# ViliamVadocz/takzero

Measured on AMD Instinct MI355X. Metric: mcts_simulations_per_s, higher is better.
Workload: dtype f16

## Files before the change

### bindings/takzero-hip-sys/src/lib.rs

```rust
#![allow(non_camel_case_types, clippy::too_many_arguments)]
use std::os::raw::{c_char, c_int, c_uint, c_void};

pub const TZ_MAX_N: c_int = 6;
pub const TZ_MAX_SQUARES: c_int = 36;
pub const TZ_MAX_ACTIONS: c_int = 512;
pub const TZ_MAX_ACTIONS_6: c_int = 1024;
pub const TZ_OK: c_int = 0;
pub const TZ_EINVAL: c_int = -1;
pub const TZ_EPARSE: c_int = -2;
pub const TZ_EDEVICE: c_int = -3;
pub const TZ_ENOMEM: c_int = -4;
pub const TZ_ECAPACITY: c_int = -5;
pub const TZ_ESTATE: c_int = -6;
pub const TZ_ENUMERIC: c_int = -7;
pub const TZ_EMPTY: c_int = 0;
pub const TZ_FLAT: c_int = 1;
pub const TZ_WALL: c_int = 2;
pub const TZ_CAP: c_int = 3;
pub const TZ_EVAL_VALUE: c_int = 0;
pub const TZ_EVAL_WIN: c_int = 1;
pub const TZ_EVAL_LOSS: c_int = 2;
pub const TZ_EVAL_DRAW: c_int = 3;
pub const TZ_TERMINAL_NONE: c_int = -1;
pub const TZ_TERMINAL_WIN: c_int = 0;
// ... 189 lines not shown
    pub fn tz_trainer_shape(t: *mut TzTrainer, board_n_out: *mut c_int, batch_out: *mut c_int, arch_out: *mut c_int) -> c_int;
    pub fn tz_trainer_load(t: *mut TzTrainer, path: *const c_char) -> c_int;
    pub fn tz_trainer_save(t: *mut TzTrainer, path: *const c_char) -> c_int;
    pub fn tz_trainer_load_weights_mem(t: *mut TzTrainer, data: *const c_void, bytes: usize) -> c_int;
    pub fn tz_trainer_get_extras(t: *mut TzTrainer, out: *mut c_void, cap: u64, bytes_out: *mut u64) -> c_int;
    pub fn tz_trainer_from_net(t: *mut TzTrainer, net: *mut TzNet) -> c_int;
    pub fn tz_trainer_to_net(t: *mut TzTrainer, net: *mut TzNet) -> c_int;
    pub fn tz_trainer_set_ensemble_targets(t: *mut TzTrainer, targets: *const f32) -> c_int;
    pub fn tz_trainer_ensemble_last(t: *mut TzTrainer, loss_out: *mut f32, values_out: *mut f32) -> c_int;
    pub fn tz_trainer_rnd_enable(t: *mut TzTrainer, on: c_int) -> c_int;
    pub fn tz_trainer_rnd_last(t: *mut TzTrainer, loss_out: *mut f32, raw_out: *mut f32) -> c_int;
    pub fn tz_trainer_rnd_activation(t: *mut TzTrainer, which: c_int, layer: c_int, out: *mut f32, out_cap: u64) -> c_int;
    pub fn tz_trainer_rnd_calibrate(t: *mut TzTrainer, early: *const TzState, n_early: c_int, late: *const TzState, n_late: c_int, apply: c_int, min_out: *mut f32, max_out: *mut f32) -> c_int;
    pub fn tz_trainer_rnd4_enable(t: *mut TzTrainer, on: c_int) -> c_int;
    pub fn tz_trainer_rnd4_last(t: *mut TzTrainer, loss_out: *mut f32, raw_out: *mut f32) -> c_int;
    pub fn tz_trainer_rnd4_activation(t: *mut TzTrainer, which: c_int, layer: c_int, out: *mut f32, out_cap: u64) -> c_int;
    pub fn tz_trainer_rnd4_calibrate(t: *mut TzTrainer, early: *const TzState, n_early: c_int, late: *const TzState, n_late: c_int, apply: c_int, min_out: *mut f32, max_out: *mut f32) -> c_int;
    pub fn tz_learn_create(trainer: *mut TzTrainer, half_komi: c_int, seed: u64, selfplay_forced_uses: c_int, reanalyze_forced_uses: c_int, out: *mut *mut TzLearn) -> c_int;
    pub fn tz_learn_destroy(l: *mut TzLearn) -> c_int;
    pub fn tz_learn_feed(l: *mut TzLearn, which: c_int, path: *const c_char, model_steps: c_int, added_out: *mut u64) -> c_int;
    pub fn tz_learn_add_lines(l: *mut TzLearn, which: c_int, text: *const c_char, len: u64, model_steps: c_int, added_out: *mut u64) -> c_int;
    pub fn tz_learn_buffer_len(l: *mut TzLearn, which: c_int, len_out: *mut u64) -> c_int;
    pub fn tz_learn_step(l: *mut TzLearn, using_reanalyze: c_int, train_ube: c_int, augment: c_int, losses_out: *mut f32) -> c_int;
    pub fn tz_learn_last_batch(l: *mut TzLearn, states_out: *mut TzState, policy_out: *mut f32, mask_out: *mut u8, value_out: *mut f32, ube_out: *mut f32) -> c_int;
    pub fn tz_learn_run(l: *mut TzLearn, directory: *const c_char, starting_steps: i64, steps: i64, min_selfplay: c_int, min_reanalyze: c_int, steps_before_reanalyze: i64, read_interval_s: f64, sleep_s: f64, wait_limit_s: f64, on_step: Option<unsafe extern "C" fn(*mut c_void, i64, *const f32, *const TzState, c_int) -> c_int>, user: *mut c_void, model_steps_out: *mut i64) -> c_int;
    pub fn tz_learn_set_save_points(l: *mut TzLearn, steps_per_save: c_int, steps_per_checkpoint: c_int, hash_net: *mut TzNet) -> c_int;
    pub fn tz_learn_set_rnd(l: *mut TzLearn, train_rnd: c_int, early: *const TzState, n_early: c_int, late: *const TzState, n_late: c_int, calibrate_every: c_int) -> c_int;
    pub fn tz_learn_rnd_reference(search: *mut TzSearch, seed: u64, n_early: c_int, early_ply: c_int, n_late: c_int, late_ply: c_int, early_out: *mut TzState, late_out: *mut TzState) -> c_int;
    pub fn tz_device_math(op: c_int, a: *const f32, b: *const f32, out: *mut f32, n: c_int) -> c_int;
    pub fn tz_debug_conv_bench(net: *mut TzNet, variant: c_int, positions: c_int, iters: c_int, ms_out: *mut f32) -> c_int;
    pub fn tz_debug_tower_bench(net: *mut TzNet, variant: c_int, positions: c_int, iters: c_int, ms_out: *mut f32) -> c_int;
    pub fn tz_debug_hash_bench(net: *mut TzNet, batch: c_int, states: *const TzState, iters: c_int, ms_out: *mut f32) -> c_int;
    pub fn tz_debug_rnd4_bench(net: *mut TzNet, batch: c_int, states: *const TzState, iters: c_int, ms_out: *mut f32) -> c_int;
    pub fn tz_debug_net_clock(net: *mut TzNet, mhz_out: *mut f64, tower_us_out: *mut f64) -> c_int;
    pub fn tz_debug_net_stamps(net: *mut TzNet, out: *mut u64, max_groups: c_int, groups_out: *mut c_int) -> c_int;
}
```

### include/takzero_hip.h

```cpp
#ifndef TAKZERO_HIP_H
#define TAKZERO_HIP_H

#include <stddef.h>
#include <stdint.h>

#ifdef __cplusplus
extern "C" {
#endif

#define TZ_MAX_N 6
#define TZ_MAX_SQUARES 36
#define TZ_MAX_ACTIONS 512
#define TZ_MAX_ACTIONS_6 1024

#define TZ_OK 0
#define TZ_EINVAL (-1)
#define TZ_EPARSE (-2)
#define TZ_EDEVICE (-3)
#define TZ_ENOMEM (-4)
#define TZ_ECAPACITY (-5)
#define TZ_ESTATE (-6)
#define TZ_ENUMERIC (-7)

#define TZ_EMPTY 0
// ... 220 lines not shown
int tz_trainer_rnd_activation(tz_trainer* t, int which, int layer, float* out, uint64_t out_cap);
int tz_trainer_rnd_calibrate(tz_trainer* t, const tz_state* early, int n_early, const tz_state* late, int n_late, int apply,
                             float* min_out, float* max_out);

int tz_trainer_rnd4_enable(tz_trainer* t, int on);
int tz_trainer_rnd4_last(tz_trainer* t, float* loss_out, float* raw_out );
int tz_trainer_rnd4_activation(tz_trainer* t, int which , int layer, float* out, uint64_t out_cap);
int tz_trainer_rnd4_calibrate(tz_trainer* t, const tz_state* early, int n_early, const tz_state* late, int n_late, int apply,
                              float* min_out, float* max_out);

typedef struct tz_learn tz_learn;
int tz_learn_create(tz_trainer* trainer, int half_komi, uint64_t seed, int selfplay_forced_uses, int reanalyze_forced_uses,
                    tz_learn** out);
int tz_learn_destroy(tz_learn* l);
int tz_learn_feed(tz_learn* l, int which, const char* path, int model_steps, uint64_t* added_out);
int tz_learn_add_lines(tz_learn* l, int which, const char* text, uint64_t len, int model_steps, uint64_t* added_out);
int tz_learn_buffer_len(tz_learn* l, int which, uint64_t* len_out);
int tz_learn_step(tz_learn* l, int using_reanalyze, int train_ube, int augment, float* losses_out);
int tz_learn_last_batch(tz_learn* l, tz_state* states_out, float* policy_out, uint8_t* mask_out, float* value_out, float* ube_out);
int tz_learn_run(tz_learn* l, const char* directory, int64_t starting_steps, int64_t steps, int min_selfplay, int min_reanalyze,
                 int64_t steps_before_reanalyze, double read_interval_s, double sleep_s, double wait_limit_s,
                 int (*on_step)(void*, int64_t, const float*, const tz_state*, int), void* user, int64_t* model_steps_out);
int tz_learn_set_save_points(tz_learn* l, int steps_per_save, int steps_per_checkpoint, tz_net* hash_net);
int tz_learn_set_rnd(tz_learn* l, int train_rnd, const tz_state* early, int n_early, const tz_state* late, int n_late,
                     int calibrate_every);
int tz_learn_rnd_reference(tz_search* search, uint64_t seed, int n_early, int early_ply, int n_late, int late_ply,
                           tz_state* early_out, tz_state* late_out);

int tz_device_math(int op, const float* a, const float* b, float* out, int n);
int tz_debug_conv_bench(tz_net* net, int variant, int positions, int iters, float* ms_out);
int tz_debug_tower_bench(tz_net* net, int variant, int positions, int iters, float* ms_out);
int tz_debug_hash_bench(tz_net* net, int batch, const tz_state* states, int iters, float* ms_out);
int tz_debug_rnd4_bench(tz_net* net, int batch, const tz_state* states, int iters, float* ms_out);
int tz_debug_net_clock(tz_net* net, double* mhz_out, double* tower_us_out);
int tz_debug_net_stamps(tz_net* net, unsigned long long* out, int max_groups, int* groups_out);

#ifdef __cplusplus
}
#endif
#endif
```

### takzero_amd/_lib.py

```python
import ctypes as C
import os

import numpy as np

HERE = os.path.dirname(os.path.abspath(__file__))
LIB_PATH = os.path.join(HERE, "libtakzero_hip.so")
MAX_SQ = 36

STATE_DTYPE = np.dtype([
    ("colors", np.uint64, (MAX_SQ,)), ("height", np.uint8, (MAX_SQ,)), ("top", np.uint8, (MAX_SQ,)),
    ("stones", np.uint8, (2,)), ("caps", np.uint8, (2,)), ("to_move", np.uint8), ("n", np.uint8),
    ("half_komi", np.int8), ("pad0", np.uint8), ("ply", np.uint16), ("reversible_plies", np.uint16),
], align=True)
ROOT_INFO_DTYPE = np.dtype([
    ("visit_count", np.uint32), ("n_children", np.uint32), ("eval_tag", np.uint8),
    ("is_terminal_env", np.uint8), ("ply", np.uint16), ("eval_bits", np.uint32),
    ("std_dev", np.float32), ("logit", np.float32), ("probability", np.float32)], align=True)
assert STATE_DTYPE.itemsize == 376 and ROOT_INFO_DTYPE.itemsize == 28

SYMBOLS = [
    "tz_last_error", "tz_version", "tz_device_count", "tz_state_from_tps", "tz_state_to_tps", "tz_move_to_ptn",
    "tz_move_from_ptn", "tz_policy_size", "tz_input_channels", "tz_net_create", "tz_net_load_weights",
    "tz_net_load_weights_mem", "tz_net_destroy", "tz_net_eval", "tz_net_encode", "tz_net_forward_raw", "tz_net_hash_indices", "tz_net_load_bitset", "tz_net_save_bitset",
    "tz_search_create", "tz_search_destroy", "tz_search_set_positions", "tz_search_get_positions",
    "tz_search_new_openings", "tz_search_simulate", "tz_search_apply_noise", "tz_search_root_info",
    "tz_search_root_children", "tz_search_node", "tz_search_select_best_actions", "tz_search_improved_policy", "tz_search_ube_target",
    "tz_search_step", "tz_search_restart_terminal", "tz_search_gumbel_sh", "tz_search_counters", "tz_search_sync", "tz_search_pool_usage",
    "tz_search_profile", "tz_device_math", "tz_debug_conv_bench", "tz_debug_tower_bench", "tz_debug_hash_bench", "tz_debug_rnd4_bench", "tz_net_ensemble_values", "tz_net_rnd_raw", "tz_net_load_prepare", "tz_net_load_commit", "tz_net_load_discard", "tz_debug_net_clock", "tz_debug_net_stamps", "tz_search_terminal_details", "tz_search_play_moves",
    "tz_trainer_set_ensemble_targets", "tz_trainer_ensemble_last", "tz_trainer_create", "tz_trainer_destroy", "tz_trainer_tensor_count", "tz_trainer_tensor_info",
    "tz_trainer_set_tensor", "tz_trainer_get_tensor", "tz_trainer_step", "tz_trainer_outputs", "tz_trainer_activation",
    "tz_format_targets", "tz_parse_targets", "tz_search_improved_policy_each", "tz_search_shape",
    "tz_selfplay_create", "tz_selfplay_destroy", "tz_selfplay_play_move", "tz_selfplay_counters", "tz_selfplay_take_text",
    "tz_selfplay_run", "tz_reanalyze_create", "tz_reanalyze_destroy", "tz_reanalyze_feed", "tz_reanalyze_iterate",
    "tz_reanalyze_take_text", "tz_reanalyze_run", "tz_compete", "tz_puzzle_benchmark", "tz_search_pool_overflows", "tz_trainer_shape",
    "tz_net_init_random", "tz_net_load_partial", "tz_net_save", "tz_net_clone", "tz_net_get_tensor", "tz_weights_convert", "tz_net_tensor_count", "tz_net_tensor_info",
    "tz_comm_unique_id", "tz_comm_rendezvous_id", "tz_comm_create_rccl", "tz_comm_create_fs", "tz_comm_destroy", "tz_comm_info",
    "tz_comm_all_gather", "tz_comm_take", "tz_comm_broadcast", "tz_comm_barrier", "tz_net_broadcast", "tz_selfplay_set_comm", "tz_selfplay_exchange",
    "tz_trainer_load", "tz_trainer_save", "tz_trainer_load_weights_mem", "tz_trainer_get_extras", "tz_trainer_from_net", "tz_trainer_to_net", "tz_learn_set_save_points",
    "tz_learn_create", "tz_learn_destroy", "tz_learn_feed", "tz_learn_add_lines", "tz_learn_buffer_len", "tz_learn_step", "tz_learn_run", "tz_learn_last_batch",
    "tz_search_simulate_batch", "tz_search_principal_variation", "tz_search_batch_profile",
    "tz_search_set_selection", "tz_search_get_selection",
    "tz_trainer_rnd_enable", "tz_trainer_rnd_last", "tz_trainer_rnd_activation", "tz_trainer_rnd_calibrate", "tz_learn_set_rnd",
    "tz_trainer_rnd4_enable", "tz_trainer_rnd4_last", "tz_trainer_rnd4_activation", "tz_trainer_rnd4_calibrate",
    "tz_learn_rnd_reference",
]

_lib = None


class TakzeroError(RuntimeError):
    def __init__(self, code, msg):
        super().__init__("libtakzero_hip error %d: %s" % (code, msg))
        self.code = code


def load():
    global _lib
    if _lib is not None:
        return _lib
    if not os.path.exists(LIB_PATH):
        try:
# ... 53 lines not shown
    lib.tz_search_set_positions.argtypes = [vp, ci, vp, vp]
    lib.tz_search_get_positions.argtypes = [vp, vp]
    lib.tz_search_new_openings.argtypes = [vp, vp]
    lib.tz_search_simulate.argtypes = [vp, vp, ci]
    lib.tz_search_simulate_batch.argtypes = [vp, vp, ci, ci]
    lib.tz_search_batch_profile.argtypes = [vp] + [C.POINTER(C.c_double)] * 3 + [C.POINTER(C.c_uint64)]
    lib.tz_search_set_selection.argtypes = [vp, ci]
    lib.tz_search_get_selection.argtypes = [vp, C.POINTER(ci)]
    lib.tz_search_principal_variation.argtypes = [vp, ci, vp, ci, C.POINTER(ci)]
    lib.tz_search_apply_noise.argtypes = [vp, vp, ci, cf]
    lib.tz_search_root_info.argtypes = [vp, vp]
    lib.tz_search_root_children.argtypes = [vp, ci] + [vp] * 7
    lib.tz_search_node.argtypes = [vp, ci, vp, ci, vp, ci] + [vp] * 7
    lib.tz_search_select_best_actions.argtypes = [vp, vp]
    lib.tz_search_improved_policy.argtypes = [vp, cf, ci, vp]
    lib.tz_search_improved_policy_each.argtypes = [vp, vp, ci, vp]
    lib.tz_search_ube_target.argtypes = [vp, cf, vp]
    lib.tz_search_step.argtypes = [vp, vp]
    lib.tz_search_restart_terminal.argtypes = [vp, vp, vp]
    lib.tz_search_gumbel_sh.argtypes = [vp, vp, ci, ci, vp, ci, vp]
    lib.tz_search_counters.argtypes = [vp, C.POINTER(C.c_uint64), C.POINTER(C.c_uint64)]
    lib.tz_search_sync.argtypes = [vp]
    lib.tz_search_pool_overflows.argtypes = [vp, C.POINTER(C.c_uint64)]
    lib.tz_search_pool_usage.argtypes = [vp, C.POINTER(C.c_uint32), C.POINTER(C.c_uint32)]
    lib.tz_search_profile.argtypes = [vp, ci, C.POINTER(C.c_double), C.POINTER(C.c_uint64), C.POINTER(C.c_double),
                                      C.POINTER(C.c_uint64)]
    lib.tz_search_terminal_details.argtypes = [vp, vp, vp]
    lib.tz_search_play_moves.argtypes = [vp, vp, vp]
    lib.tz_device_math.argtypes = [ci, vp, vp, vp, ci]
    lib.tz_debug_conv_bench.argtypes = [vp, ci, ci, ci, C.POINTER(C.c_float)]
    lib.tz_debug_tower_bench.argtypes = [vp, ci, ci, ci, C.POINTER(C.c_float)]
    lib.tz_debug_hash_bench.argtypes = [vp, ci, vp, ci, C.POINTER(C.c_float)]
    lib.tz_debug_rnd4_bench.argtypes = [vp, ci, vp, ci, C.POINTER(C.c_float)]
    lib.tz_net_ensemble_values.argtypes = [vp, ci, vp, vp]
    lib.tz_net_rnd_raw.argtypes = [vp, ci, vp, vp]
    lib.tz_debug_net_clock.argtypes = [vp, C.POINTER(C.c_double), C.POINTER(C.c_double)]
    lib.tz_debug_net_stamps.argtypes = [vp, C.POINTER(C.c_uint64), C.c_int, C.POINTER(C.c_int)]
    lib.tz_net_load_prepare.argtypes = [vp, C.c_char_p, C.POINTER(vp)]
    lib.tz_net_load_commit.argtypes = [vp, vp]
    lib.tz_net_load_discard.argtypes = [vp]
    lib.tz_format_targets.argtypes = [ci, ci, vp, vp, vp, vp, ci, vp, vp, vp, C.c_uint64, C.POINTER(C.c_uint64)]
    lib.tz_parse_targets.argtypes = [vp, C.c_uint64, ci, ci, ci, ci, vp, vp, vp, vp, vp, vp, C.POINTER(C.c_int32),
                                     C.POINTER(C.c_uint64), C.POINTER(C.c_int32)]
    lib.tz_search_shape.argtypes = [vp] + [C.POINTER(ci)] * 4
    lib.tz_selfplay_create.argtypes = [vp, ci, C.c_uint64, ci, ci, ci, ci, C.POINTER(vp)]
    lib.tz_selfplay_destroy.argtypes = [vp]
    lib.tz_selfplay_play_move.argtypes = [vp]
    lib.tz_selfplay_counters.argtypes = [vp] + [C.POINTER(C.c_uint64)] * 3
    lib.tz_selfplay_take_text.argtypes = [vp, ci, vp, C.c_uint64, C.POINTER(C.c_uint64)]
    lib.tz_selfplay_run.argtypes = [vp, C.c_char_p, ci, ci, C.c_char_p, vp, vp, C.c_double]
    lib.tz_reanalyze_create.argtypes = [vp, ci, C.c_uint64, ci, ci, ci, ci, C.POINTER(vp)]
    lib.tz_reanalyze_destroy.argtypes = [vp]
    lib.tz_reanalyze_feed.argtypes = [vp, C.c_char_p, C.POINTER(C.c_uint64), C.POINTER(C.c_uint64)]
    lib.tz_reanalyze_iterate.argtypes = [vp]
    lib.tz_reanalyze_take_text.argtypes = [vp, vp, C.c_uint64, C.POINTER(C.c_uint64)]
    lib.tz_reanalyze_run.argtypes = [vp, C.c_char_p, ci, ci, C.c_char_p, vp, vp, C.c_double]
    lib.tz_compete.argtypes = [vp, vp, vp, cf, cf, C.c_uint64, ci, ci, ci, vp]
    lib.tz_puzzle_benchmark.argtypes = [vp, vp, vp, ci, ci, C.c_uint64, ci, ci, vp]
    lib.tz_trainer_shape.argtypes = [vp] + [C.POINTER(ci)] * 3
    lib.tz_learn_create.argtypes = [vp, ci, C.c_uint64, ci, ci, C.POINTER(vp)]
    lib.tz_learn_destroy.argtypes = [vp]
    lib.tz_learn_feed.argtypes = [vp, ci, C.c_char_p, ci, C.POINTER(C.c_uint64)]
    lib.tz_learn_add_lines.argtypes = [vp, ci, vp, C.c_uint64, ci, C.POINTER(C.c_uint64)]
    lib.tz_learn_buffer_len.argtypes = [vp, ci, C.POINTER(C.c_uint64)]
    lib.tz_learn_step.argtypes = [vp, ci, ci, ci, vp]
    lib.tz_learn_last_batch.argtypes = [vp, vp, vp, vp, vp, vp]
# ... 31 lines not shown
```

### takzero_amd/csrc/tz_nn.h

```cpp
#pragma once
#include <string>
#include <vector>

#include "tz_engine.h"
#include "tz_ot.h"

struct ConvW {
    int taps = 0, cin = 0, cin_pad = 0, cout = 0, cout_pad = 0;
    uint16_t* w_mfma = nullptr;
    uint16_t* w_lo = nullptr;
    unsigned char* w8 = nullptr;
    float c8_scale = 0.0f;
    float* w_f32 = nullptr;
    float* bias = nullptr;
};

struct tz_net {
    int n = 0, nn = 0, arch = 0, device = 0, precision = 0, blocks = 0;
    int cin = 0, cin_pad = 0, pol_ch = 0, pol_stride = 0, ppt = 0;
    bool loaded = false, has_rnd = false, has_hash = false, has_ens = false;
    bool has_rnd_tower = false;
    TensorStore store;
    uint64_t capture_gen = 0;
    ConvW conv_in, policy;
    std::vector<ConvW> res;
    uint16_t* tower_w = nullptr;
    uint16_t* tower_w_lo = nullptr;
    unsigned char* tower_w8 = nullptr;
    float* c8_scales = nullptr;
    float* tower_bias = nullptr;
    float* heads = nullptr;
    ConvW rnd[2][3];
    uint16_t* rndw[3] = {nullptr, nullptr, nullptr};
    float* rndb[3] = {nullptr, nullptr, nullptr};
    float rnd_min = 0.0f, rnd_max = 1.0f;
    float* simhash = nullptr;
    uint32_t* bitset = nullptr;
    float* ens_w = nullptr;
    uint16_t* rnd4_w = nullptr;
    float *rnd4_wf = nullptr, *rnd4_bias = nullptr, *rnd4_ln = nullptr;
    int max_batch = 0;
    void *act_a = nullptr, *act_b = nullptr, *act_c = nullptr;
    float* planes = nullptr;
    float* policy_out = nullptr;
    float *value = nullptr, *ube = nullptr, *variance = nullptr, *aux = nullptr;
    void *rnd_in = nullptr, *rnd_h1 = nullptr, *rnd_h2 = nullptr;
    float* rnd_out = nullptr;
    float* ens_act = nullptr;
    float* ens_values = nullptr;
    void* seeds = nullptr;
    void* xch = nullptr;
    unsigned* xch_count = nullptr;
    bool eval_split = false;
    hipStream_t stream_rnd = nullptr;
    hipEvent_t ev_in = nullptr, ev_rnd = nullptr;
    hipStream_t stream = nullptr;
    void* dbg_buf = nullptr;
    int dbg_groups = 0;
    void* eval_host = nullptr;
    void* eval_dev = nullptr;
    size_t eval_bytes = 0;
    hipEvent_t ev0 = nullptr, ev1 = nullptr;
    std::vector<std::pair<hipEvent_t, hipEvent_t>> conv_events;
    bool profile = false;
    double conv_ms = 0.0;
    uint64_t conv_launches = 0;
};

int tz_net_ensure_batch(tz_net* net, int batch);
void tz_net_invalidate_captures(tz_net* net);
int tz_net_forward_device(tz_net* net, const tz_state* states_dev, const int32_t* game_index_dev,
                          const int32_t* count_dev, int count_host, int max_positions, hipStream_t st, NetOut* out);
int tz_nn_encode_planes(int n, int cin, const tz_state* states_dev, int count, float* planes_dev, hipStream_t st);
```

### takzero_amd/csrc/tz_nn.hip

```cpp
#include "tz_nn.h"
#include "tz_fp8.h"
#include "tz_fp6.h"
#include "tz_math.h"
#include <type_traits>
#include "tz_ot.h"
#include "tz_nn_rnd4.h"

#include <algorithm>
#include <cmath>
#include <cstdio>
#include <cstdlib>
#include <cstring>
#include <atomic>
#include <map>
#include <memory>
#include <mutex>
#include <thread>

int tz_nn_launch_split(int sp, int n, const void* net_args, int max_positions, hipStream_t st);
int tz_nn_launch_c6(int n, const void* net_args, int max_positions, hipStream_t st);
size_t tz_nn_c6_seed_bytes(int n, int max_positions);

namespace {

// ... 342 lines not shown
#pragma unroll
                        for (int j = 0; j < RN; j++) bnext[j] = wload(tap, slice * 8 + kc + 1, j);
                    } else if (tap + 1 < TAPS) {
#pragma unroll
                        for (int j = 0; j < RN; j++) bnext[j] = wload(tap + 1, slice * 8, j);
                    }
#pragma unroll
                    for (int rt = 0; rt < RT; rt++) {
                        const ex8 av = *reinterpret_cast<const ex8*>(lds + abase[rt] + kc * KSTEP);
#pragma unroll
                        for (int j = 0; j < RN; j++)
                            acc[rt][j] = Elem<ET>::mfma(bcur[j], av, acc[rt][j]);
                    }
                }
            }
        }
    }

#pragma unroll
    for (int j = 0; j < RN; j++) {
        const int cbase = (ct0 + j) * 16 + q * 4;
        const f32x4 bias = *reinterpret_cast<const f32x4*>(a.bias + (size_t)blockIdx.z * a.bias_z + cbase);
#pragma unroll
        for (int rt = 0; rt < RT; rt++) {
            const int r = rt * 16 + lr;
            if (r >= valid_rows) continue;
            f32x4 v = acc[rt][j] + bias;
            const size_t o = (size_t)blockIdx.z * a.out_z + (m0 + r) * a.out_stride + cbase;
            if (a.has_res) {
                const ex4 rv = *reinterpret_cast<const ex4*>(reinterpret_cast<const uint16_t*>(a.residual) + o);
#pragma unroll
                for (int k = 0; k < 4; k++) v[k] += (float)rv[k];
            }
            if (a.relu) {
#pragma unroll
                for (int k = 0; k < 4; k++) v[k] = v[k] > 0.f ? v[k] : 0.f;
            }
            if (a.out_f32) {
                *reinterpret_cast<f32x4*>(reinterpret_cast<float*>(a.out) + o) = v;
            } else {
                ex4 ov;
#pragma unroll
                for (int k = 0; k < 4; k++) ov[k] = Elem<ET>::cvt(v[k]);
                *reinterpret_cast<ex4*>(reinterpret_cast<uint16_t*>(a.out) + o) = ov;
            }
        }
    }
}

struct TowerArgs {
    const uint16_t* in;
    uint16_t* out;
    const uint16_t* w;
    const float* bias;
    const int32_t* count_dev;
    int count_host;
    int nlayers;
};

template <int NB, int P, int OPT = 0, typename ET = __bf16>
__global__ __launch_bounds__(512, 2) void tower_mfma_kernel(TowerArgs a) {
    typedef typename Elem<ET>::x8 ex8;
    typedef typename Elem<ET>::x4 ex4;
    constexpr int RN = 2, TAPS = 9, LAYOUT = 1, NT = 512;
    constexpr int NN = NB * NB, ROWS = P * NN, RT = (ROWS + 15) / 16, LROWS = RT * 16 + 8, ZROW = RT * 16;
    constexpr int PLANE = LROWS * LDS_ROWB, KSTEP = PLANE;
// ... 2701 lines not shown
}

__host__ __device__ constexpr int ppt_small(int nb) { return nb == 1 ? 64 : nb == 3 ? 7 : nb == 4 ? 6 : nb == 5 ? 4 : 3; }

int conv_cfg() {
    static int cfg = -1;
    if (cfg < 0) {
        const char* e = getenv("TZ_CONV_CFG");
        cfg = e ? atoi(e) : 0;
    }
    return cfg;
}

template <int NB, int P, int NW, int RN, int TAPS, bool FROM_STATE, bool SINGLE, int ABL = 0, int LAYOUT = 1, typename ET = __bf16, int OCC = 2>
int launch_conv(const ConvArgs& a, int max_positions, int n_blocks_y, hipStream_t st) {
    constexpr int NN = NB * NB, RT = (P * NN + 15) / 16, LROWS = RT * 16 + 8;
    const size_t smem = LdsImg<LAYOUT>::bytes(LROWS);
    auto kern = conv_mfma_kernel<NB, P, RN, TAPS, FROM_STATE, ABL, SINGLE, NW, LAYOUT, ET, OCC>;
    static bool attr_done[64] = {};
    int attr_dev = 0;
    TZ_HIP(hipGetDevice(&attr_dev));
    bool& attr_set = attr_done[attr_dev & 63];
    if (!attr_set) {
        TZ_HIP(hipFuncSetAttribute(reinterpret_cast<const void*>(kern), hipFuncAttributeMaxDynamicSharedMemorySize, (int)smem));
        attr_set = true;
    }
    dim3 grid((max_positions + P - 1) / P, n_blocks_y, a.groups > 1 ? a.groups : 1);
    hipLaunchKernelGGL(kern, grid, dim3(NW * 64), smem, st, a);
    hipError_t e = hipGetLastError();
    if (e != hipSuccess) return tz_fail(TZ_EDEVICE, std::string("conv launch: ") + hipGetErrorString(e));
    return TZ_OK;
}

int linear_grouped_bf16(int precision, const uint16_t* w, const float* bias, int groups, int cin_pad, int cout_pad, const void* in,
                        int in_stride, int in_z, void* out, int out_stride, int out_z, bool relu, bool out_f32,
                        const int32_t* count_dev, int count_host, int max_positions, hipStream_t st) {
    ConvArgs a;
    memset(&a, 0, sizeof a);
    a.in = in;
    a.count_dev = count_dev;
    a.count_host = count_host;
    a.w = w;
    a.bias = bias;
    a.out = out;
    a.cin_pad = cin_pad;
    a.kc_total = cin_pad / 32;
    a.ct_total = cout_pad / 16;
    a.out_stride = out_stride;
    a.cin_real = cin_pad;
    a.relu = relu;
    a.out_f32 = out_f32;
    a.in_stride = in_stride;
    a.groups = groups;
    a.in_z = in_z;
    a.w_z_frags = a.kc_total * a.ct_total;
    a.bias_z = cout_pad;
    a.out_z = out_z;
    if (max_positions <= 128) {
        if (prec_is_f16(precision)) return launch_conv<1, 32, 8, 2, 1, false, false, 0, 1, _Float16>(a, max_positions, cout_pad / 256, st);
        return launch_conv<1, 32, 8, 2, 1, false, false>(a, max_positions, cout_pad / 256, st);
    }
    if (prec_is_f16(precision)) return launch_conv<1, 128, 8, 2, 1, false, false, 0, 1, _Float16>(a, max_positions, cout_pad / 256, st);
    return launch_conv<1, 128, 8, 2, 1, false, false>(a, max_positions, cout_pad / 256, st);
}

template <int NB, typename ET>
int conv_board(const ConvArgs& a, int cout_pad, bool from_state, int max_positions, hipStream_t st) {
    constexpr int PA = ppt_for(NB), PB = ppt_small(NB);
    const bool wide = cout_pad % 256 == 0;
    const int by = wide ? cout_pad / 256 : cout_pad / 128;
    if (conv_cfg() == 0) {
        if (from_state) return launch_conv<NB, PA, 8, 2, 9, true, false, 0, 1, ET>(a, max_positions, by, st);
        if (wide) return launch_conv<NB, PA, 8, 2, 9, false, true, 0, 1, ET>(a, max_positions, by, st);
        return launch_conv<NB, PA, 8, 1, 9, false, true, 0, 1, ET>(a, max_positions, by, st);
    }
    if (from_state) return launch_conv<NB, PB, 4, 4, 9, true, false, 0, 1, ET>(a, max_positions, by, st);
    if (wide) return launch_conv<NB, PB, 4, 4, 9, false, true, 0, 1, ET>(a, max_positions, by, st);
    return launch_conv<NB, PB, 4, 2, 9, false, true, 0, 1, ET>(a, max_positions, by, st);
}

template <typename ET>
int conv_dispatch(int n, bool board, const ConvArgs& a, int cout_pad, bool from_state, int max_positions, hipStream_t st) {
    if (!board) return launch_conv<1, 64, 8, 2, 1, false, false, 0, 1, ET>(a, max_positions, cout_pad / 256, st);
    switch (n) {
        case 3: return conv_board<3, ET>(a, cout_pad, from_state, max_positions, st);
        case 4: return conv_board<4, ET>(a, cout_pad, from_state, max_positions, st);
        case 5: return conv_board<5, ET>(a, cout_pad, from_state, max_positions, st);
        case 6: return conv_board<6, ET>(a, cout_pad, from_state, max_positions, st);
    }
    return tz_fail(TZ_EINVAL, "conv: unsupported board size");
}

int conv_bf16(tz_net* net, const ConvW& L, const void* in, const tz_state* states, const int32_t* gidx,
              const int32_t* count_dev, int count_host, int max_positions, const void* residual, void* out,
              int out_stride, bool relu, bool out_f32, bool board, hipStream_t st) {
    ConvArgs a;
// ... 390 lines not shown
                     (void**)&net->value, (void**)&net->ube, (void**)&net->variance, (void**)&net->aux,
                     &net->rnd_in, &net->rnd_h1, &net->rnd_h2, (void**)&net->rnd_out, &net->seeds, (void**)&net->ens_act, (void**)&net->ens_values};
    for (auto b : bufs) {
        if (*b) (void)hipFree(*b);
        *b = nullptr;
    }
    const size_t esz = net->precision != TZ_PREC_F32 ? 2 : 4;
    const size_t rows = (size_t)batch * net->nn;
    TZ_HIP(hipMalloc(&net->act_a, rows * FILTERS * esz));
    TZ_HIP(hipMalloc(&net->act_b, rows * FILTERS * esz));
    TZ_HIP(hipMalloc(&net->act_c, rows * FILTERS * esz));
    TZ_HIP(hipMalloc(&net->planes, rows * net->cin * sizeof(float)));
    TZ_HIP(hipMalloc(&net->policy_out, rows * net->pol_stride * sizeof(float)));
    TZ_HIP(hipMalloc(&net->value, batch * sizeof(float)));
    TZ_HIP(hipMalloc(&net->ube, batch * sizeof(float)));
    TZ_HIP(hipMalloc(&net->variance, batch * sizeof(float)));
    TZ_HIP(hipMalloc(&net->aux, batch * sizeof(float)));
    if (net->precision == TZ_PREC_F16C6) TZ_HIP(hipMalloc(&net->seeds, tz_nn_c6_seed_bytes(net->n, batch)));
    if (net->has_ens) {
        TZ_HIP(hipMalloc(&net->ens_act, rows * FILTERS * sizeof(float)));
        TZ_HIP(hipMalloc(&net->ens_values, (size_t)batch * ENS_HEADS * sizeof(float)));
    }
    if (net->has_rnd) {
        const size_t in_pad = (size_t)(net->cin * net->nn + 31) / 32 * 32;
        TZ_HIP(hipMalloc(&net->rnd_in, (size_t)batch * in_pad * esz));
        TZ_HIP(hipMalloc(&net->rnd_h1, (size_t)batch * 2048 * esz));
        TZ_HIP(hipMalloc(&net->rnd_h2, (size_t)batch * 2048 * esz));
        TZ_HIP(hipMalloc(&net->rnd_out, (size_t)2 * batch * 512 * sizeof(float)));
    }
    net->max_batch = batch;
    return TZ_OK;
}

int tz_net_forward_device(tz_net* net, const tz_state* states, const int32_t* gidx, const int32_t* count_dev,
                          int count_host, int max_positions, hipStream_t st, NetOut* out) {
    if (!net->loaded) return tz_fail(TZ_ESTATE, "network has no weights loaded");
    if (max_positions > net->max_batch) return tz_fail(TZ_EINVAL, "forward: batch exceeds the network's buffers");
    int rc;
    const bool bf = net->precision != TZ_PREC_F32;
    const int nn = net->nn;
    const bool need_planes = !bf;
    if (need_planes && (rc = encode(net, states, gidx, count_dev, count_host, max_positions, st))) return rc;
    void *x = net->act_a, *t = net->act_b, *y = net->act_c;
    const void* last = nullptr;
    const bool split = prec_is_split(net->precision);
    const int rnd_in_pad = (net->cin * nn + 31) / 32 * 32;
    const bool rnd_ahead = net->eval_split && net->has_rnd && bf && net->n == 5 && net->stream_rnd;
    auto rnd_mlp = [&](hipStream_t rs) -> int {
        const bool fused_wrote_it = net->blocks > 0 && net->tower_w && (net_fused_mode() == 2 || split) && net_fused_writes_rnd_input(net);
        switch (net->n) {
            case 5:
                if (fused_wrote_it) break;
                if (prec_is_f16(net->precision))
                    rnd_prep_state_kernel<5, _Float16><<<max_positions, 64, 0, rs>>>(states, gidx, count_dev, count_host, net->cin, rnd_in_pad, (_Float16*)net->rnd_in);
                else
                    rnd_prep_state_kernel<5, __bf16><<<max_positions, 64, 0, rs>>>(states, gidx, count_dev, count_host, net->cin, rnd_in_pad, (__bf16*)net->rnd_in);
                break;
            default: return tz_fail(TZ_EINVAL, "RND is a net5 (5x5) feature");
        }
        float* o = net->rnd_out;
        if ((rc = linear_grouped_bf16(net->precision, net->rndw[0], net->rndb[0], 1, rnd_in_pad, 2048, net->rnd_in, rnd_in_pad, 0, net->rnd_h1, 2048, 0,
                                      true, false, count_dev, count_host, max_positions, rs)))
            return rc;
        if ((rc = linear_grouped_bf16(net->precision, net->rndw[1], net->rndb[1], 2, 1024, 1024, net->rnd_h1, 2048, 1024, net->rnd_h2, 2048, 1024,
                                      true, false, count_dev, count_host, max_positions, rs)))
            return rc;
        if ((rc = linear_grouped_bf16(net->precision, net->rndw[2], net->rndb[2], 2, 1024, 512, net->rnd_h2, 2048, 1024, o, 1024, 512, false, true,
                                      count_dev, count_host, max_positions, rs)))
            return rc;
        return TZ_OK;
    };

    if (split && !(net->blocks > 0 && (net->tower_w_lo || net->tower_w8)))
        return tz_fail(TZ_EINVAL, "forward: TZ_PREC_F16X2 / TZ_PREC_F16C8 / TZ_PREC_F16C6 need a network with at least one residual block");
    if (bf && net->blocks > 0 && net->tower_w && (net_fused_mode() == 2 || split)) {
        hipEvent_t e0 = nullptr, e1 = nullptr;
        if (net->profile) {
            TZ_HIP(hipEventCreate(&e0));
            TZ_HIP(hipEventCreate(&e1));
            TZ_HIP(hipEventRecord(e0, st));
        }
        if (rnd_ahead) {
            TZ_HIP(hipEventRecord(net->ev_in, st));
            TZ_HIP(hipStreamWaitEvent(net->stream_rnd, net->ev_in, 0));
            if ((rc = rnd_mlp(net->stream_rnd))) return rc;
            TZ_HIP(hipEventRecord(net->ev_rnd, net->stream_rnd));
        }
        if ((rc = net_fused(net, states, gidx, count_dev, count_host, max_positions, st))) return rc;
        if (net->profile) {
            TZ_HIP(hipEventRecord(e1, st));
            net->conv_events.push_back({e0, e1});
            net->conv_launches += 1;
        }
    } else if (bf) {
        if ((rc = conv_bf16(net, net->conv_in, nullptr, states, gidx, count_dev, count_host, max_positions, nullptr, x, FILTERS,
                            true, false, true, st)))
            return rc;
        if (net->blocks > 0 && net->tower_w && net_fused_mode() >= 1) {
            hipEvent_t e0 = nullptr, e1 = nullptr;
            if (net->profile) {
                TZ_HIP(hipEventCreate(&e0));
                TZ_HIP(hipEventCreate(&e1));
// ... 993 lines not shown

int tz_debug_rnd4_bench(tz_net* net, int batch, const tz_state* states, int iters, float* ms_out) {
    if (!net || !states || !ms_out || batch <= 0 || iters <= 0) return tz_fail(TZ_EINVAL, "tz_debug_rnd4_bench: bad argument");
    if (!net->has_rnd_tower || !net->loaded) return tz_fail(TZ_ESTATE, "tz_debug_rnd4_bench: not a loaded TZ_ARCH_NET4_RND network");
    tz_state* dstates = nullptr;
    int rc = net_upload_states(net, batch, states, &dstates);
    if (rc) return rc;
    hipStream_t st = net->stream;
    hipEvent_t e0 = nullptr, e1 = nullptr;
    float ms = 0.f;
    hipError_t e = hipEventCreate(&e0);
    if (e == hipSuccess) e = hipEventCreate(&e1);
    if (e == hipSuccess) e = hipMemsetAsync(net->ube, 0, (size_t)batch * sizeof(float), st);
    auto launch = [&]() {
        return tz_nn_launch_rnd4(net->precision == TZ_PREC_F32, dstates, nullptr, nullptr, batch, batch, net->rnd4_w, net->rnd4_wf, net->rnd4_bias,
                                 net->rnd4_ln, net->ube, net->rnd_min, net->rnd_max, net->aux, net->variance, st);
    };
    for (int i = 0; i < 2 && e == hipSuccess && !rc; i++) rc = launch();
    if (e == hipSuccess && !rc) e = hipEventRecord(e0, st);
    for (int i = 0; i < iters && e == hipSuccess && !rc; i++) rc = launch();
    if (e == hipSuccess && !rc) e = hipEventRecord(e1, st);
    if (e == hipSuccess && !rc) e = hipEventSynchronize(e1);
    if (e == hipSuccess && !rc) e = hipEventElapsedTime(&ms, e0, e1);
    if (e == hipSuccess && !rc) e = hipGetLastError();
    if (e0) (void)hipEventDestroy(e0);
    if (e1) (void)hipEventDestroy(e1);
    (void)hipFree(dstates);
    if (rc) return rc;
    if (e != hipSuccess) return tz_fail(TZ_EDEVICE, std::string("tz_debug_rnd4_bench: ") + hipGetErrorString(e));
    *ms_out = ms / iters;
    return TZ_OK;
}

int tz_net_load_bitset(tz_net* net, const char* path) {
    if (!net || !path) return tz_fail(TZ_EINVAL, "tz_net_load_bitset: null argument");
    if (!net->has_hash) return tz_fail(TZ_ESTATE, "tz_net_load_bitset: not a SimHash network");
    TZ_HIP(hipSetDevice(net->device));
    FILE* f = fopen(path, "rb");
    if (!f) return tz_fail(TZ_EPARSE, std::string("tz_net_load_bitset: cannot open ") + path);
    const size_t total = (size_t)1 << 29, chunk = (size_t)1 << 26;
    std::vector<unsigned char> buf(chunk);
    uint32_t* staging = nullptr;
    if (hipMalloc(&staging, total) != hipSuccess) {
        fclose(f);
        return tz_fail(TZ_ENOMEM, "tz_net_load_bitset: cannot allocate the staging set");
    }
    size_t done = 0;
    while (done < total) {
        const size_t rd = fread(buf.data(), 1, chunk, f);
        if (rd != chunk || hipMemcpy((unsigned char*)staging + done, buf.data(), chunk, hipMemcpyHostToDevice) != hipSuccess) break;
        done += chunk;
    }
    fclose(f);
    if (done != total) {
        (void)hipFree(staging);
        return tz_fail(TZ_EPARSE, "tz_net_load_bitset: file is not 2^32 bits");
    }
    TZ_HIP(hipStreamSynchronize(net->stream));
    tz_net_invalidate_captures(net);
    (void)hipFree(net->bitset);
    net->bitset = staging;
    return TZ_OK;
}

int tz_net_save_bitset(tz_net* net, const char* path) {
    if (!net || !path) return tz_fail(TZ_EINVAL, "tz_net_save_bitset: null argument");
// ... 95 lines not shown
```

Baseline: 1.476 million.

## Add ring-buffered LDS pipelined kernel for RND MLP linear layers

Adds a dedicated rnd_linear_kernel for the RND MLP's large linear layers. It double-buffers input slices in LDS, prefetches weight fragments several k-steps ahead through buffer loads, and overlaps global fetches with MFMA accumulation. By default it replaces the generic 1x1 conv path for the 128-row case and picks a 64- or 128-row tile depending on grid height. The old conv path and a deeper prefetch variant remain selectable through an environment variable. It also adds a debug bench with event probes, at the cost of extra code and register pressure that could reduce occupancy.

Result: no change. 1.480 million, median of 5 (+0.3%).

```diff
diff --git a/bindings/takzero-hip-sys/src/lib.rs b/bindings/takzero-hip-sys/src/lib.rs
--- a/bindings/takzero-hip-sys/src/lib.rs
+++ b/bindings/takzero-hip-sys/src/lib.rs
@@ -245,6 +245,7 @@
     pub fn tz_debug_tower_bench(net: *mut TzNet, variant: c_int, positions: c_int, iters: c_int, ms_out: *mut f32) -> c_int;
     pub fn tz_debug_hash_bench(net: *mut TzNet, batch: c_int, states: *const TzState, iters: c_int, ms_out: *mut f32) -> c_int;
     pub fn tz_debug_rnd4_bench(net: *mut TzNet, batch: c_int, states: *const TzState, iters: c_int, ms_out: *mut f32) -> c_int;
+    pub fn tz_debug_rnd_linear_bench(net: *mut TzNet, batch: c_int, states: *const TzState, iters: c_int, ms_out: *mut f32) -> c_int;
     pub fn tz_debug_net_clock(net: *mut TzNet, mhz_out: *mut f64, tower_us_out: *mut f64) -> c_int;
     pub fn tz_debug_net_stamps(net: *mut TzNet, out: *mut u64, max_groups: c_int, groups_out: *mut c_int) -> c_int;
 }
diff --git a/include/takzero_hip.h b/include/takzero_hip.h
--- a/include/takzero_hip.h
+++ b/include/takzero_hip.h
@@ -276,6 +276,7 @@
 int tz_debug_tower_bench(tz_net* net, int variant, int positions, int iters, float* ms_out);
 int tz_debug_hash_bench(tz_net* net, int batch, const tz_state* states, int iters, float* ms_out);
 int tz_debug_rnd4_bench(tz_net* net, int batch, const tz_state* states, int iters, float* ms_out);
+int tz_debug_rnd_linear_bench(tz_net* net, int batch, const tz_state* states, int iters, float* ms_out);
 int tz_debug_net_clock(tz_net* net, double* mhz_out, double* tower_us_out);
 int tz_debug_net_stamps(tz_net* net, unsigned long long* out, int max_groups, int* groups_out);
 
diff --git a/takzero_amd/_lib.py b/takzero_amd/_lib.py
--- a/takzero_amd/_lib.py
+++ b/takzero_amd/_lib.py
@@ -26,7 +26,7 @@
     "tz_search_new_openings", "tz_search_simulate", "tz_search_apply_noise", "tz_search_root_info",
     "tz_search_root_children", "tz_search_node", "tz_search_select_best_actions", "tz_search_improved_policy", "tz_search_ube_target",
     "tz_search_step", "tz_search_restart_terminal", "tz_search_gumbel_sh", "tz_search_counters", "tz_search_sync", "tz_search_pool_usage",
-    "tz_search_profile", "tz_device_math", "tz_debug_conv_bench", "tz_debug_tower_bench", "tz_debug_hash_bench", "tz_debug_rnd4_bench", "tz_net_ensemble_values", "tz_net_rnd_raw", "tz_net_load_prepare", "tz_net_load_commit", "tz_net_load_discard", "tz_debug_net_clock", "tz_debug_net_stamps", "tz_search_terminal_details", "tz_search_play_moves",
+    "tz_search_profile", "tz_device_math", "tz_debug_conv_bench", "tz_debug_tower_bench", "tz_debug_hash_bench", "tz_debug_rnd4_bench", "tz_debug_rnd_linear_bench", "tz_net_ensemble_values", "tz_net_rnd_raw", "tz_net_load_prepare", "tz_net_load_commit", "tz_net_load_discard", "tz_debug_net_clock", "tz_debug_net_stamps", "tz_search_terminal_details", "tz_search_play_moves",
     "tz_trainer_set_ensemble_targets", "tz_trainer_ensemble_last", "tz_trainer_create", "tz_trainer_destroy", "tz_trainer_tensor_count", "tz_trainer_tensor_info",
     "tz_trainer_set_tensor", "tz_trainer_get_tensor", "tz_trainer_step", "tz_trainer_outputs", "tz_trainer_activation",
     "tz_format_targets", "tz_parse_targets", "tz_search_improved_policy_each", "tz_search_shape",
@@ -146,6 +146,7 @@
     lib.tz_debug_tower_bench.argtypes = [vp, ci, ci, ci, C.POINTER(C.c_float)]
     lib.tz_debug_hash_bench.argtypes = [vp, ci, vp, ci, C.POINTER(C.c_float)]
     lib.tz_debug_rnd4_bench.argtypes = [vp, ci, vp, ci, C.POINTER(C.c_float)]
+    lib.tz_debug_rnd_linear_bench.argtypes = [vp, ci, vp, ci, C.POINTER(C.c_float)]
     lib.tz_net_ensemble_values.argtypes = [vp, ci, vp, vp]
     lib.tz_net_rnd_raw.argtypes = [vp, ci, vp, vp]
     lib.tz_debug_net_clock.argtypes = [vp, C.POINTER(C.c_double), C.POINTER(C.c_double)]
diff --git a/takzero_amd/csrc/tz_nn.h b/takzero_amd/csrc/tz_nn.h
--- a/takzero_amd/csrc/tz_nn.h
+++ b/takzero_amd/csrc/tz_nn.h
@@ -55,6 +55,7 @@
     hipStream_t stream_rnd = nullptr;
     hipEvent_t ev_in = nullptr, ev_rnd = nullptr;
     hipStream_t stream = nullptr;
+    hipEvent_t rnd_probe[2] = {nullptr, nullptr};
     void* dbg_buf = nullptr;
     int dbg_groups = 0;
     void* eval_host = nullptr;
diff --git a/takzero_amd/csrc/tz_nn.hip b/takzero_amd/csrc/tz_nn.hip
--- a/takzero_amd/csrc/tz_nn.hip
+++ b/takzero_amd/csrc/tz_nn.hip
@@ -398,6 +398,133 @@
 #pragma unroll
                 for (int k = 0; k < 4; k++) v[k] += (float)rv[k];
             }
+            if (a.relu) {
+#pragma unroll
+                for (int k = 0; k < 4; k++) v[k] = v[k] > 0.f ? v[k] : 0.f;
+            }
+            if (a.out_f32) {
+                *reinterpret_cast<f32x4*>(reinterpret_cast<float*>(a.out) + o) = v;
+            } else {
+                ex4 ov;
+#pragma unroll
+                for (int k = 0; k < 4; k++) ov[k] = Elem<ET>::cvt(v[k]);
+                *reinterpret_cast<ex4*>(reinterpret_cast<uint16_t*>(a.out) + o) = ov;
+            }
+        }
+    }
+}
+
+template <typename ET, int TM, int OCC, int AHEAD = 2>
+__global__ __launch_bounds__(512, OCC) void rnd_linear_kernel(ConvArgs a) {
+    typedef typename Elem<ET>::x8 ex8;
+    typedef typename Elem<ET>::x4 ex4;
+    constexpr int RT = TM / 16, RN = 2, NT = 512;
+    constexpr int PLANE = TM * LDS_ROWB, BUF = 4 * PLANE;
+    constexpr int NLOAD = TM * 16 / NT;
+    static_assert(TM % 32 == 0 && NLOAD >= 1 && 2 * BUF <= 65536 && (BUF & (BUF - 1)) == 0 && AHEAD >= 1 && AHEAD <= 3, "rnd_linear_kernel: tile");
+    extern __shared__ __attribute__((aligned(16))) unsigned char lds[];
+    const int count = a.count_dev ? *a.count_dev : a.count_host;
+    const int pos0 = blockIdx.x * TM;
+    if (pos0 >= count) return;
+    const int tid = threadIdx.x, lane = tid & 63;
+    const int wave = __builtin_amdgcn_readfirstlane(tid >> 6);
+    const int q = lane >> 4, lr = lane & 15;
+    const int valid_rows = min(TM, count - pos0);
+    const size_t m0 = (size_t)pos0;
+    const int ct0 = (blockIdx.y * 8 + wave) * RN;
+    const int kt = a.kc_total, nslices = (kt + 3) >> 2;
+    const __amdgpu_buffer_rsrc_t wrsrc = __builtin_amdgcn_make_buffer_rsrc(
+        const_cast<uint16_t*>(a.w), 0, (a.groups > 1 ? a.groups * a.w_z_frags : a.kc_total * a.ct_total) * 1024, 0x00020000);
+    const int lane16 = lane * 16;
+    const int wfrag0 = (int)blockIdx.z * a.w_z_frags + ct0;
+    auto wload = [&](int kc, int j) -> ex8 {
+        const u32x4 r = __builtin_amdgcn_raw_buffer_load_b128(wrsrc, lane16, (wfrag0 + kc * a.ct_total + j) * 1024, 0);
+        return __builtin_bit_cast(ex8, r);
+    };
+    const uint16_t* in = reinterpret_cast<const uint16_t*>(a.in) + (size_t)blockIdx.z * a.in_z;
+    uint4 stage[NLOAD];
+    auto fetch_slice = [&](int slice) {
+        const int left = a.cin_pad - slice * 128;
+#pragma unroll
+        for (int i = 0; i < NLOAD; i++) {
+            const int id = tid + i * NT, row = (id >> 6) * 4 + ((id >> 2) & 3), ci = ((id >> 4) & 3) * 4 + (id & 3);
+            stage[i] = make_uint4(0, 0, 0, 0);
+            if (row < valid_rows && ci * 8 < left) stage[i] = *reinterpret_cast<const uint4*>(in + (m0 + row) * a.in_stride + slice * 128 + ci * 8);
+        }
+    };
+    auto store_slice = [&](int buf_off) {
+#pragma unroll
+        for (int i = 0; i < NLOAD; i++) {
+            const int id = tid + i * NT, row = (id >> 6) * 4 + ((id >> 2) & 3), plane = (id >> 4) & 3;
+            *reinterpret_cast<uint4*>(lds + buf_off + plane * PLANE + row * LDS_ROWB + lds_piece(row, id & 3)) = stage[i];
+        }
+    };
+    fetch_slice(0);
+    ex8 bq[4][RN];
+#pragma unroll
+    for (int i = 0; i < AHEAD; i++)
+#pragma unroll
+        for (int j = 0; j < RN; j++) bq[i][j] = wload(min(i, kt - 1), j);
+    f32x4 acc[RT][RN];
+#pragma unroll
+    for (int rt = 0; rt < RT; rt++)
+#pragma unroll
+        for (int j = 0; j < RN; j++) acc[rt][j] = f32x4{0.f, 0.f, 0.f, 0.f};
+    int abase[RT];
+#pragma unroll
+    for (int rt = 0; rt < RT; rt++) abase[rt] = (rt * 16 + lr) * LDS_ROWB + lds_piece(rt * 16 + lr, q);
+    store_slice(0);
+    fetch_slice(1);
+    __syncthreads();
+    ex8 av[RT];
+#pragma unroll
+    for (int rt = 0; rt < RT; rt++) av[rt] = *reinterpret_cast<const ex8*>(lds + abase[rt]);
+    auto kstep = [&](int kc, int p, bool barrier) __attribute__((always_inline)) {
+        const int kn = min(kc + AHEAD, kt - 1);
+#pragma unroll
+        for (int j = 0; j < RN; j++) bq[(p + AHEAD) & 3][j] = wload(kn, j);
+        __builtin_amdgcn_sched_barrier(0);
+        if (barrier) {
+            __syncthreads();
+#pragma unroll
+            for (int rt = 0; rt < RT; rt++) abase[rt] ^= BUF;
+        }
+#pragma unroll
+        for (int rt = 0; rt < RT; rt++) {
+#pragma unroll
+            for (int j = 0; j < RN; j++) acc[rt][j] = Elem<ET>::mfma(bq[p][j], av[rt], acc[rt][j]);
+            av[rt] = *reinterpret_cast<const ex8*>(lds + abase[rt] + ((p + 1) & 3) * PLANE);
+        }
+    };
+    const int nfull = kt >> 2;
+    int wbuf = BUF;
+    for (int slice = 0; slice < nfull; slice++) {
+#pragma unroll
+        for (int p = 0; p < 4; p++) {
+            kstep(slice * 4 + p, p, p == 3);
+            if (p == 1) {
+                if (slice + 1 < nslices) {
+                    store_slice(wbuf);
+                    fetch_slice(slice + 2);
+                }
+                wbuf ^= BUF;
+            }
+        }
+    }
+#pragma unroll
+    for (int p = 0; p < 3; p++)
+        if (p < (kt & 3)) kstep(nfull * 4 + p, p, false);
+
+#pragma unroll
+    for (int j = 0; j < RN; j++) {
+        const int cbase = (ct0 + j) * 16 + q * 4;
+        const f32x4 bias = *reinterpret_cast<const f32x4*>(a.bias + (size_t)blockIdx.z * a.bias_z + cbase);
+#pragma unroll
+        for (int rt = 0; rt < RT; rt++) {
+            const int r = rt * 16 + lr;
+            if (r >= valid_rows) continue;
+            f32x4 v = acc[rt][j] + bias;
+            const size_t o = (size_t)blockIdx.z * a.out_z + (m0 + r) * a.out_stride + cbase;
             if (a.relu) {
 #pragma unroll
                 for (int k = 0; k < 4; k++) v[k] = v[k] > 0.f ? v[k] : 0.f;
@@ -3165,6 +3292,53 @@
     return TZ_OK;
 }
 
+enum { RND_LINEAR_RING = 0, RND_LINEAR_CONV = 1, RND_LINEAR_CONV64 = 2, RND_LINEAR_RING3 = 3 };
+int rnd_linear_form() {
+    static const int form = [] {
+        const char* e = getenv("TZ_RND_LINEAR");
+        if (e && !strcmp(e, "conv")) return (int)RND_LINEAR_CONV;
+        if (e && !strcmp(e, "conv64")) return (int)RND_LINEAR_CONV64;
+        if (e && !strcmp(e, "ring3")) return (int)RND_LINEAR_RING3;
+        return (int)RND_LINEAR_RING;
+    }();
+    return form;
+}
+
+template <typename ET, int TM, int OCC, int AHEAD = 2>
+int launch_rnd_linear(const ConvArgs& a, int max_positions, int n_blocks_y, hipStream_t st) {
+    constexpr size_t smem = 2 * 4 * (size_t)TM * LDS_ROWB;
+    auto kern = rnd_linear_kernel<ET, TM, OCC, AHEAD>;
+    static bool attr_done[64] = {};
+    int attr_dev = 0;
+    TZ_HIP(hipGetDevice(&attr_dev));
+    bool& attr_set = attr_done[attr_dev & 63];
+    if (!attr_set) {
+        TZ_HIP(hipFuncSetAttribute(reinterpret_cast<const void*>(kern), hipFuncAttributeMaxDynamicSharedMemorySize, (int)smem));
+        attr_set = true;
+    }
+    dim3 grid((max_positions + TM - 1) / TM, n_blocks_y, a.groups > 1 ? a.groups : 1);
+    hipLaunchKernelGGL(kern, grid, dim3(512), smem, st, a);
+    hipError_t e = hipGetLastError();
+    if (e != hipSuccess) return tz_fail(TZ_EDEVICE, std::string("rnd linear launch: ") + hipGetErrorString(e));
+    return TZ_OK;
+}
+
+template <typename ET>
+int rnd_linear_dispatch(const ConvArgs& a, int max_positions, int cout_pad, hipStream_t st) {
+    const int by = cout_pad / 256;
+    switch (rnd_linear_form()) {
+        case RND_LINEAR_CONV: return launch_conv<1, 128, 8, 2, 1, false, false, 0, 1, ET>(a, max_positions, by, st);
+        case RND_LINEAR_CONV64: return launch_conv<1, 64, 8, 2, 1, false, false, 0, 1, ET, 4>(a, max_positions, by, st);
+    }
+    const bool tall = by * (a.groups > 1 ? a.groups : 1) >= 8;
+    if (rnd_linear_form() == RND_LINEAR_RING3) {
+        if (tall) return launch_rnd_linear<ET, 128, 2, 3>(a, max_positions, by, st);
+        return launch_rnd_linear<ET, 64, 2, 3>(a, max_positions, by, st);
+    }
+    if (tall) return launch_rnd_linear<ET, 128, 2>(a, max_positions, by, st);
+    return launch_rnd_linear<ET, 64, 2>(a, max_positions, by, st);
+}
+
 int linear_grouped_bf16(int precision, const uint16_t* w, const float* bias, int groups, int cin_pad, int cout_pad, const void* in,
                         int in_stride, int in_z, void* out, int out_stride, int out_z, bool relu, bool out_f32,
                         const int32_t* count_dev, int count_host, int max_positions, hipStream_t st) {
@@ -3193,8 +3367,8 @@
         if (prec_is_f16(precision)) return launch_conv<1, 32, 8, 2, 1, false, false, 0, 1, _Float16>(a, max_positions, cout_pad / 256, st);
         return launch_conv<1, 32, 8, 2, 1, false, false>(a, max_positions, cout_pad / 256, st);
     }
-    if (prec_is_f16(precision)) return launch_conv<1, 128, 8, 2, 1, false, false, 0, 1, _Float16>(a, max_positions, cout_pad / 256, st);
-    return launch_conv<1, 128, 8, 2, 1, false, false>(a, max_positions, cout_pad / 256, st);
+    if (prec_is_f16(precision)) return rnd_linear_dispatch<_Float16>(a, max_positions, cout_pad, st);
+    return rnd_linear_dispatch<__bf16>(a, max_positions, cout_pad, st);
 }
 
 template <int NB, typename ET>
@@ -3651,6 +3825,21 @@
     return TZ_OK;
 }
 
+static int rnd_linear_layer(tz_net* net, int layer, const int32_t* count_dev, int count_host, int max_positions, hipStream_t rs) {
+    const int rnd_in_pad = (net->cin * net->nn + 31) / 32 * 32;
+    switch (layer) {
+        case 0:
+            return linear_grouped_bf16(net->precision, net->rndw[0], net->rndb[0], 1, rnd_in_pad, 2048, net->rnd_in, rnd_in_pad, 0, net->rnd_h1, 2048, 0,
+                                       true, false, count_dev, count_host, max_positions, rs);
+        case 1:
+            return linear_grouped_bf16(net->precision, net->rndw[1], net->rndb[1], 2, 1024, 1024, net->rnd_h1, 2048, 1024, net->rnd_h2, 2048, 1024,
+                                       true, false, count_dev, count_host, max_positions, rs);
+        default:
+            return linear_grouped_bf16(net->precision, net->rndw[2], net->rndb[2], 2, 1024, 512, net->rnd_h2, 2048, 1024, net->rnd_out, 1024, 512, false, true,
+                                       count_dev, count_host, max_positions, rs);
+    }
+}
+
 int tz_net_forward_device(tz_net* net, const tz_state* states, const int32_t* gidx, const int32_t* count_dev,
                           int count_host, int max_positions, hipStream_t st, NetOut* out) {
     if (!net->loaded) return tz_fail(TZ_ESTATE, "network has no weights loaded");
@@ -3677,16 +3866,10 @@
                 break;
             default: return tz_fail(TZ_EINVAL, "RND is a net5 (5x5) feature");
         }
-        float* o = net->rnd_out;
-        if ((rc = linear_grouped_bf16(net->precision, net->rndw[0], net->rndb[0], 1, rnd_in_pad, 2048, net->rnd_in, rnd_in_pad, 0, net->rnd_h1, 2048, 0,
-                                      true, false, count_dev, count_host, max_positions, rs)))
-            return rc;
-        if ((rc = linear_grouped_bf16(net->precision, net->rndw[1], net->rndb[1], 2, 1024, 1024, net->rnd_h1, 2048, 1024, net->rnd_h2, 2048, 1024,
-                                      true, false, count_dev, count_host, max_positions, rs)))
-            return rc;
-        if ((rc = linear_grouped_bf16(net->precision, net->rndw[2], net->rndb[2], 2, 1024, 512, net->rnd_h2, 2048, 1024, o, 1024, 512, false, true,
-                                      count_dev, count_host, max_positions, rs)))
-            return rc;
+        if (net->rnd_probe[0]) TZ_HIP(hipEventRecord(net->rnd_probe[0], rs));
+        for (int layer = 0; layer < 3; layer++)
+            if ((rc = rnd_linear_layer(net, layer, count_dev, count_host, max_positions, rs))) return rc;
+        if (net->rnd_probe[1]) TZ_HIP(hipEventRecord(net->rnd_probe[1], rs));
         return TZ_OK;
     };
 
@@ -4746,6 +4929,48 @@
     return TZ_OK;
 }
 
+int tz_debug_rnd_linear_bench(tz_net* net, int batch, const tz_state* states, int iters, float* ms_out) {
+    if (!net || !states || !ms_out || batch <= 0 || iters <= 0) return tz_fail(TZ_EINVAL, "tz_debug_rnd_linear_bench: bad argument");
+    if (!net->has_rnd || !net->loaded || net->precision == TZ_PREC_F32) return tz_fail(TZ_ESTATE, "tz_debug_rnd_linear_bench: needs a loaded net5 on a 16-bit path");
+    tz_state* dstates = nullptr;
+    int rc = net_upload_states(net, batch, states, &dstates);
+    if (rc) return rc;
+    hipStream_t st = net->stream;
+    hipEvent_t e0 = nullptr, e1 = nullptr;
+    NetOut o;
+    hipError_t e = hipEventCreate(&e0);
+    if (e == hipSuccess) e = hipEventCreate(&e1);
+    for (int i = 0; i < 2 && e == hipSuccess && !rc; i++) rc = tz_net_forward_device(net, dstates, nullptr, nullptr, batch, batch, st, &o);
+    for (int layer = 0; layer < 3 && e == hipSuccess && !rc; layer++) {
+        float ms = 0.f;
+        e = hipEventRecord(e0, st);
+        for (int i = 0; i < iters && e == hipSuccess && !rc; i++) rc = rnd_linear_layer(net, layer, nullptr, batch, batch, st);
+        if (e == hipSuccess && !rc) e = hipEventRecord(e1, st);
+        if (e == hipSuccess && !rc) e = hipEventSynchronize(e1);
+        if (e == hipSuccess && !rc) e = hipEventElapsedTime(&ms, e0, e1);
+        ms_out[layer] = ms / iters;
+    }
+    double sum = 0.0;
+    net->rnd_probe[0] = e0;
+    net->rnd_probe[1] = e1;
+    for (int i = 0; i < iters && e == hipSuccess && !rc; i++) {
+        float ms = 0.f;
+        rc = tz_net_forward_device(net, dstates, nullptr, nullptr, batch, batch, st, &o);
+        if (!rc) e = hipStreamSynchronize(st);
+        if (e == hipSuccess && !rc) e = hipEventElapsedTime(&ms, e0, e1);
+        sum += ms;
+    }
+    net->rnd_probe[0] = net->rnd_probe[1] = nullptr;
+    if (e == hipSuccess && !rc) e = hipGetLastError();
+    if (e0) (void)hipEventDestroy(e0);
+    if (e1) (void)hipEventDestroy(e1);
+    (void)hipFree(dstates);
+    if (rc) return rc;
+    if (e != hipSuccess) return tz_fail(TZ_EDEVICE, std::string("tz_debug_rnd_linear_bench: ") + hipGetErrorString(e));
+    ms_out[3] = (float)(sum / iters);
+    return TZ_OK;
+}
+
 int tz_net_load_bitset(tz_net* net, const char* path) {
     if (!net || !path) return tz_fail(TZ_EINVAL, "tz_net_load_bitset: null argument");
     if (!net->has_hash) return tz_fail(TZ_ESTATE, "tz_net_load_bitset: not a SimHash network");
```
